# davrempe/humor

Hardware: AMD Instinct MI355X
Metric: fitting closure evaluations/s (stage-3 objective fwd+bwd), batch=32 seq=60 per GPU (higher is better)
Workload: dtype f32

## Files before the change

### humor_amd/csrc/rollout.hip

```cpp
#include <string.h>

#include <algorithm>
#include <list>
#include <unordered_map>
#include <vector>

#include "rollout_persist.h"
#include "rot_math.h"

namespace ha {

constexpr int D_IN = 339, D_STATE = 348, ZD = 48, NJT = 22, NBODY = 21;
template <int ROTW>
struct RawLayout {
  static constexpr int ROOT = 6, RVEL = 6 + ROTW, BODY = 9 + ROTW, JNT = 9 + 22 * ROTW, JVEL = JNT + 66, CONT = JVEL + 66, D = CONT + 9;
};
static_assert(RawLayout<3>::D == 216 && RawLayout<6>::D == 282 && RawLayout<9>::D == 348, "decoder output widths of the three representations");
constexpr int D_INP = 340;
constexpr int SLICE = 64;
constexpr int MAXL = 8;

typedef float f32x16 __attribute__((ext_vector_type(16)));
typedef float vf4 __attribute__((ext_vector_type(4)));

__device__ __forceinline__ size_t qoff(int c) { return (size_t)(c >> 2) * 128 + (c & 3); }

int g_layer_finish = 1;
int g_gemm_rm = 0;
int g_gemm_ks = 2;
int g_rollout_groups = 0;
int g_rollout_persist = 1;
int g_rollout_persist_bwd = 1;
int g_rollout_pipe = 1;
int g_rollout_pipe_bwd = 1;
int g_rollout_persist_inject = 0;

enum class Path : int { chain = 0, one_launch = 1, one_launch_lean = 2 };

struct CallPlan {
  Path path = Path::chain;
  bool piped = false;
  int ngroups = 1, rows_per_group = 0;
  size_t group_floats = 0;
  const float* g_z_add = nullptr;
};

struct PackedLayer {
  int Cin = 0, skip = 0, Nout = 0;
  int nslices_f = 0, main_slices = 0, ntiles_f = 0, Nout_pad = 0;
  int nslices_b = 0, ntiles_b = 0, Nin_pad = 0;
  int group = 0;
  float* Wf = nullptr;
  float* Wb = nullptr;
  float* bias = nullptr;
  float* gamma = nullptr;
  float* beta = nullptr;
};

}

struct ha_humor_net {
  int device = 0;
  int n_dec = 0, n_pri = 0;
  int rotw = 3;
  bool delta = true;
  ha::PackedLayer dec[ha::MAXL], pri[ha::MAXL];
  ha::PersistNet* persist = nullptr;
  struct StashRec { ha::CallPlan plan; int B, S, knobs; std::list<const void*>::iterator age; };
  static constexpr size_t MAX_STASH_RECS = 65536;
  mutable std::unordered_map<const void*, StashRec> stash_recs;
  mutable std::list<const void*> stash_age;
};

namespace ha {

struct LayerTask {
  const float* Wp; const float* bias;
  int ntiles, nslices, main_slices, Nout, Nout_pad;
  const float* src; int nsplit_src; int Csrc;
  const float* skip; int skip_dim;
  int mode;
  const float* gamma; const float* beta; int group; float inv_group;
// ... 253 lines not shown
    v[0] = a0.x; v[1] = a0.y; v[2] = a0.z; v[3] = a0.w; v[4] = a1.x; v[5] = a1.y; v[6] = a1.z; v[7] = a1.w;
  };
  float x[8], da[8];
  if (T.mode == 1) load8(T.src, T.nsplit_src, T.Csrc, x);
  else { load8(T.src, T.nsplit_src, T.Csrc, da); load8(T.hsrc, T.nsplit_h, T.Ch, x); }
  const float gam[8] = {g0.x, g0.y, g0.z, g0.w, g1.x, g1.y, g1.z, g1.w};
  const float bet[8] = {e0.x, e0.y, e0.z, e0.w, e1.x, e1.y, e1.z, e1.w};
  const int per = T.group == SLICE ? 8 : 4, o0 = T.group == SLICE ? 0 : (oct & 4);
  const float inv_n = 1.0f / (float)T.group;
  auto row_sum = [&](int pass, float v) {
    s_red[pass][row][oct] = v;
    __syncthreads();
    float t = 0.f;
    for (int k = 0; k < per; ++k) t += s_red[pass][row][o0 + k];
    return t;
  };
  float p1 = 0.f;
#pragma unroll
  for (int i = 0; i < 8; ++i) p1 += x[i];
  const float mu = row_sum(0, p1) * inv_n;
  float p2 = 0.f;
#pragma unroll
  for (int i = 0; i < 8; ++i) { const float d = x[i] - mu; p2 = fmaf(d, d, p2); }
  const float rstd = rsqrtf(row_sum(1, p2) * inv_n + 1e-5f);
  float out[8];
  if (T.mode == 1) {
#pragma unroll
    for (int i = 0; i < 8; ++i) out[i] = fmaxf((x[i] - mu) * rstd * gam[i] + bet[i], 0.f);
  } else {
    float xh[8], dxh[8], m1 = 0.f, m2 = 0.f;
#pragma unroll
    for (int i = 0; i < 8; ++i) {
      xh[i] = (x[i] - mu) * rstd;
      const float y = xh[i] * gam[i] + bet[i];
      dxh[i] = (y > 0.f ? da[i] : 0.f) * gam[i];
      m1 += dxh[i];
      m2 = fmaf(dxh[i], xh[i], m2);
    }
    m1 = row_sum(2, m1) * inv_n;
    m2 = row_sum(3, m2) * inv_n;
#pragma unroll
    for (int i = 0; i < 8; ++i) out[i] = rstd * (dxh[i] - m1 - xh[i] * m2);
  }
  float* d = F.dst[ti] + (size_t)rt * (T.main_slices * SLICE) * 32 + (size_t)(c0 >> 2) * 128 + (size_t)row * 4;
  *reinterpret_cast<vf4*>(d) = vf4{out[0], out[1], out[2], out[3]};
  *reinterpret_cast<vf4*>(d + 128) = vf4{out[4], out[5], out[6], out[7]};
}


struct GemmTask {
  const float* Wp; const float* bias;
  int ntiles, nslices, Nout;
  const float* src; int Csrc;
  int nrt;
  int epi;
  float slope;
  const float* gamma; const float* beta; int group;
  const float* hsrc; int Ch;
  float* dst_h; float* dst_a; int Cdst;
  int nrg, nwork, per_xcd;
};

constexpr int GEMM_LDS_WAVE = 2 * 8 * 132;

template <int RM, int KS = 1, int TN = 2>
__global__ __launch_bounds__(256) void prior_gemm_kernel(GemmTask T) {
  static_assert(KS == 1 || RM == 1, "the K split is built for one row tile per wave");
  static_assert((KS == 1 || KS == 2 || KS == 4) && (TN == 1 || TN == 2), "prior_gemm_kernel: unsupported shape");
  extern __shared__ __attribute__((aligned(16))) float smem[];
  const int wave = threadIdx.x >> 6, lane = threadIdx.x & 63;
  const int w = (int)(blockIdx.x & 7) * T.per_xcd + (int)(blockIdx.x >> 3);
  if ((int)(blockIdx.x >> 3) >= T.per_xcd || w >= T.nwork) return;
  const int cb = w / T.nrg, rg = w % T.nrg;
  const int kpart = KS == 1 ? 0 : wave % KS;
  const int ct0 = KS == 1 ? (cb * 4 + wave) * TN : (cb * (4 / KS) + wave / KS) * TN;
  const bool tile_ok = ct0 < T.ntiles;
  if (KS == 1 && !tile_ok) return;
  const int ct1 = TN == 2 && ct0 + 1 < T.ntiles ? ct0 + 1 : ct0;
  int rt[RM];
#pragma unroll
  for (int m = 0; m < RM; ++m) rt[m] = rg * RM + m < T.nrt ? rg * RM + m : T.nrt - 1;

  f32x16 acc[RM][TN];
#pragma unroll
  for (int m = 0; m < RM; ++m)
#pragma unroll
    for (int c = 0; c < TN; ++c)
#pragma unroll
      for (int i = 0; i < 16; ++i) acc[m][c][i] = 0.f;

  const float* wp0 = T.Wp + (size_t)ct0 * T.nslices * 2048 + lane * 4;
  const float* wp1 = T.Wp + (size_t)ct1 * T.nslices * 2048 + lane * 4;
  auto load_b = [&](int slice, float (&b0)[32], float (&b1)[32]) {
#pragma unroll
    for (int j = 0; j < 8; ++j) {
      const vf4 u = *reinterpret_cast<const vf4*>(wp0 + (size_t)slice * 2048 + j * 256);
      b0[4 * j] = u.x; b0[4 * j + 1] = u.y; b0[4 * j + 2] = u.z; b0[4 * j + 3] = u.w;
      if (TN == 2) {
        const vf4 v = *reinterpret_cast<const vf4*>(wp1 + (size_t)slice * 2048 + j * 256);
        b1[4 * j] = v.x; b1[4 * j + 1] = v.y; b1[4 * j + 2] = v.z; b1[4 * j + 3] = v.w;
      }
    }
  };
  auto load_a = [&](int slice, float (&a)[RM][32]) {
#pragma unroll
    for (int m = 0; m < RM; ++m)
      load_frag<1>(T.src + (size_t)rt[m] * T.Csrc * 32 + (size_t)(slice * 16 + 8 * (lane >> 5)) * 128 + (size_t)(lane & 31) * 4, 0, 8, a[m]);
  };
  auto mma = [&](const float (&a)[RM][32], const float (&b0)[32], const float (&b1)[32]) {
#pragma unroll
    for (int kp = 0; kp < 32; ++kp)
#pragma unroll
      for (int m = 0; m < RM; ++m) {
        acc[m][0] = __builtin_amdgcn_mfma_f32_32x32x2f32(a[m][kp], b0[kp], acc[m][0], 0, 0, 0);
        if (TN == 2) acc[m][TN - 1] = __builtin_amdgcn_mfma_f32_32x32x2f32(a[m][kp], b1[kp], acc[m][TN - 1], 0, 0, 0);
      }
  };
  const int nfull_all = T.Csrc / SLICE < T.nslices ? T.Csrc / SLICE : T.nslices;
  const int per_part = (nfull_all + KS - 1) / KS;
  const int sbeg = KS == 1 ? 0 : (kpart * per_part < nfull_all ? kpart * per_part : nfull_all);
  const int nfull = KS == 1 ? nfull_all : ((sbeg + per_part) < nfull_all ? (sbeg + per_part) : nfull_all);
  if (nfull > sbeg && (KS == 1 || tile_ok)) {
    float aA[RM][32], bA0[32], bA1[32], aB[RM][32], bB0[32], bB1[32];
    load_b(sbeg, bA0, bA1);
    load_a(sbeg, aA);
    for (int slice = sbeg; slice < nfull; slice += 2) {
      const int s1 = slice + 1 < nfull ? slice + 1 : slice;
      load_b(s1, bB0, bB1);
      load_a(s1, aB);
      HA_SCHED_FENCE();
      mma(aA, bA0, bA1);
      HA_SCHED_FENCE();
      if (slice + 1 < nfull) {
        const int s2 = slice + 2 < nfull ? slice + 2 : slice + 1;
        load_b(s2, bA0, bA1);
        load_a(s2, aA);
        HA_SCHED_FENCE();
        mma(aB, bB0, bB1);
        HA_SCHED_FENCE();
      }
    }
  }
  if (nfull_all < T.nslices && kpart == KS - 1 && (KS == 1 || tile_ok)) {
    float a[RM][32], b0[32], b1[32];
    load_b(nfull_all, b0, b1);
#pragma unroll
    for (int m = 0; m < RM; ++m) load_frag_n<true>(T.src, 1, 0, T.Csrc, rt[m], nfull_all * SLICE, lane, a[m]);
    mma(a, b0, b1);
  }

  float* sl = smem + wave * GEMM_LDS_WAVE;
  const int row = lane & 31, hh = lane >> 5;
  const int ct = hh ? ct0 + 1 : ct0;
  const bool ct_ok = hh < TN && ct < T.ntiles;
  const int hs = hh < TN ? hh : 0;
  float gam[32], bet[32];
  if ((T.epi == 1 || T.epi == 3) && ct_ok) {
#pragma unroll
    for (int j = 0; j < 8; ++j) {
      const vf4 g4 = *reinterpret_cast<const vf4*>(T.gamma + ct * 32 + 4 * j);
      const vf4 b4 = *reinterpret_cast<const vf4*>(T.beta + ct * 32 + 4 * j);
      gam[4 * j] = g4.x; gam[4 * j + 1] = g4.y; gam[4 * j + 2] = g4.z; gam[4 * j + 3] = g4.w;
      bet[4 * j] = b4.x; bet[4 * j + 1] = b4.y; bet[4 * j + 2] = b4.z; bet[4 * j + 3] = b4.w;
    }
  } else {
#pragma unroll
    for (int k = 0; k < 32; ++k) { gam[k] = 1.f; bet[k] = 0.f; }
  }
#pragma unroll
  for (int m = 0; m < RM; ++m) {
#pragma unroll
    for (int c = 0; c < TN; ++c)
#pragma unroll
      for (int i = 0; i < 16; ++i) {
        const int r = (i & 3) + 8 * (i >> 2) + 4 * hh, col = lane & 31;
        sl[(c * 8 + (col >> 2)) * 132 + r * 4 + (col & 3)] = acc[m][c][i];
      }
    if (KS == 1) {
      __builtin_amdgcn_fence(__ATOMIC_RELEASE, "wavefront");
      __builtin_amdgcn_wave_barrier();
      __builtin_amdgcn_fence(__ATOMIC_ACQUIRE, "wavefront");
    } else {
      __syncthreads();
      if (kpart != 0) return;
    }
    float v[32];
#pragma unroll
    for (int j = 0; j < 8; ++j) {
      vf4 q = *reinterpret_cast<const vf4*>(sl + (hs * 8 + j) * 132 + row * 4);
      if (KS > 1) {
#pragma unroll
        for (int pk = 1; pk < KS; ++pk) q += *reinterpret_cast<const vf4*>(sl + pk * GEMM_LDS_WAVE + (hs * 8 + j) * 132 + row * 4);
      }
      v[4 * j] = q.x; v[4 * j + 1] = q.y; v[4 * j + 2] = q.z; v[4 * j + 3] = q.w;
    }
    if (KS == 1) {
      __builtin_amdgcn_fence(__ATOMIC_RELEASE, "wavefront");
      __builtin_amdgcn_wave_barrier();
      __builtin_amdgcn_fence(__ATOMIC_ACQUIRE, "wavefront");
    }
    const bool live = ct_ok && rg * RM + m < T.nrt;
    if (T.bias && ct_ok) {
#pragma unroll
      for (int j = 0; j < 8; ++j) {
        const vf4 b4 = *reinterpret_cast<const vf4*>(T.bias + ct * 32 + 4 * j);
        v[4 * j] += b4.x; v[4 * j + 1] += b4.y; v[4 * j + 2] += b4.z; v[4 * j + 3] += b4.w;
      }
    }
    const size_t o = (size_t)rt[m] * T.Cdst * 32 + (size_t)(ct * 8) * 128 + (size_t)row * 4;
    auto store32 = [&](float* base, const float (&x)[32]) {
#pragma unroll
      for (int j = 0; j < 8; ++j) *reinterpret_cast<vf4*>(base + o + (size_t)j * 128) = vf4{x[4 * j], x[4 * j + 1], x[4 * j + 2], x[4 * j + 3]};
    };
    if (T.epi <= 1 && live) store32(T.dst_h, v);
    if (T.epi == 4) {
#pragma unroll
      for (int k = 0; k < 32; ++k) v[k] = v[k] > 0.f ? v[k] : v[k] * T.slope;
      if (live) store32(T.dst_a, v);
    } else if (T.epi == 5) {
      const float* hp = T.hsrc + (size_t)rt[m] * T.Ch * 32 + (size_t)((ct_ok ? ct : ct0) * 8) * 128 + (size_t)row * 4;
#pragma unroll
      for (int j = 0; j < 8; ++j) {
        const vf4 q = *reinterpret_cast<const vf4*>(hp + (size_t)j * 128);
        v[4 * j] *= q.x > 0.f ? 1.f : T.slope; v[4 * j + 1] *= q.y > 0.f ? 1.f : T.slope;
        v[4 * j + 2] *= q.z > 0.f ? 1.f : T.slope; v[4 * j + 3] *= q.w > 0.f ? 1.f : T.slope;
      }
      if (live) store32(T.dst_a, v);
    } else if (T.epi == 1) {
      const float inv_n = 1.0f / (float)T.group;
      if (T.group == SLICE) gn_apply<1>(1, gam, bet, inv_n, v, v);
      else gn_apply<2>(1, gam, bet, inv_n, v, v);
      if (live) store32(T.dst_a, v);
    } else if (T.epi == 3) {
      float h[32];
      const float* hp = T.hsrc + (size_t)rt[m] * T.Ch * 32 + (size_t)((ct_ok ? ct : ct0) * 8) * 128 + (size_t)row * 4;
#pragma unroll
      for (int j = 0; j < 8; ++j) {
        const vf4 q = *reinterpret_cast<const vf4*>(hp + (size_t)j * 128);
        h[4 * j] = q.x; h[4 * j + 1] = q.y; h[4 * j + 2] = q.z; h[4 * j + 3] = q.w;
      }
      const float inv_n = 1.0f / (float)T.group;
      if (T.group == SLICE) gn_apply<1>(3, gam, bet, inv_n, h, v);
      else gn_apply<2>(3, gam, bet, inv_n, h, v);
      if (live) store32(T.dst_a, v);
    }
  }
}

struct GlueParams {
  int B, S, t, RT;
  const float* xT;
  float* xT_next;
  const float* dec_out; int dec_nsplit; int dec_pad;
  const float* pri_out; int pri_nsplit; int pri_pad;
  const float* Gs;
  float* Gs_next;
  const float* t2j;
  float* world;
  float* prior_mu; float* prior_var;
  const float* g_world;
  const float* g_prior_mu; const float* g_prior_var;
  float* g_dec_out;
  float* g_pri_out;
  const float* gx_dir_in;
  float* gx_dir_out;
  const float* gxp_pri; int gxp_pri_nsplit; int gxp_pri_pad;
  const float* gxp_dec; int gxp_dec_nsplit; int gxp_dec_pad;
  float* carry;
  const float* dz_src[MAXL]; int dz_nsplit[MAXL]; int dz_pad[MAXL]; int dz_off[MAXL]; int dz_n;
  float* g_z;
  float* g_past0;
};

__device__ __forceinline__ float tsum(const float* base, int nsplit, int RT, int C, int rt, int c, int row) {
  return base ? slab_sum(base, nsplit, RT, C, rt, c, row) : 0.f;
}

struct PredState {
  float pj[3], jv[3];
  float dB[9], Bin[9], pB[9];
  float ptrans[3], ptvel[3], prvel[3], dR[9], Rin[9], pR[9];
  float raw_aa_b[9], raw_aa_r[9];
};

template <int ROTW>
__device__ __forceinline__ void delta_rot(const float* raw, float R[9]) {
  if constexpr (ROTW == 3) rodrigues(raw, R);
  else if constexpr (ROTW == 6) rot6d_to_rotmat(raw, R);
  else rot9d_to_rotmat(raw, R);
}
template <int ROTW>
__device__ __forceinline__ void delta_rot_bwd(const float* raw, const float gR[9], float* graw) {
  if constexpr (ROTW == 3) rodrigues_bwd(raw, gR, graw);
  else if constexpr (ROTW == 6) rot6d_to_rotmat_bwd(raw, gR, graw);
  else rot9d_to_rotmat_bwd(raw, gR, graw);
}
// ... 884 lines not shown
      F.t[k] = T;
      F.dst[k] = stash + L.fin[i];
      F.nblk[k] = LL.RT * T.main_slices;
      fb += F.nblk[k];
      T.src = F.dst[k]; T.nsplit_src = 1; T.Csrc = T.main_slices * SLICE; T.mode = 0;
      T.hsrc = nullptr; T.nsplit_h = 0;
    }
    if (fb) {
      HA_LAUNCH(gn_finish_kernel, dim3(fb), dim3(256), 4 * 32 * 8 * sizeof(float), st, F);
      HA_LAUNCH_CHECK();
    }
  }
  LayerTask& T0 = LL.t[0];
  const dim3 grid(T0.ntiles, T0.nsplit_dst, LL.RT);
  T0.nblocks *= LL.RT;
  const bool lean = L.finish && T0.mode == 0 && T0.nsplit_src <= 1;
  if (lean) HA_LAUNCH((mlp_layer_kernel<4, true>), grid, dim3(256), 4 * 1024 * sizeof(float), st, LL);
  else HA_LAUNCH((mlp_layer_kernel<4, false>), grid, dim3(256), 4 * 1024 * sizeof(float), st, LL);
  HA_LAUNCH_CHECK();
  return HA_OK;
}


struct GemmPlan { int rm, tn, ks, ncb; };

static GemmPlan plan_prior_gemm(int ntiles, int nslices, int nrt, int epi, int rm_knob, int ks_knob) {
  GemmPlan P;
  P.ncb = ceil_div(ntiles, 8);
  P.rm = rm_knob == 1 || rm_knob == 2 ? rm_knob : ((nrt / 2) * P.ncb >= 2 * 256 ? 2 : 1);
  P.tn = 2;
  P.ks = 1;
  const bool split_on = ks_knob == 2 || ks_knob == 3;
  if (!split_on || P.rm == 2) return P;
  const bool force = ks_knob == 3;
  if (!force && P.ncb * nrt * 4 > 512) return P;
  const bool gn = epi == 1 || epi == 3;
  constexpr int SIMDS = 1024;
  int best = ceil_div(ceil_div(ntiles, 2) * nrt, SIMDS) * nslices * 2;
  if (force) best = nslices * 2;
  for (int tn = 2; tn >= (gn ? 2 : 1); --tn)
    for (int ks = 1; ks <= 4; ks *= 2) {
      if (ks > 1 && nslices < 2 * ks) continue;
      const int waves = ceil_div(ntiles, tn) * nrt * ks;
      if (!force && waves > 2 * SIMDS) continue;
      const int chain = ceil_div(nslices, ks) * tn;
      const int cost = force ? chain : ceil_div(waves, SIMDS) * chain;
      if (cost < best || (force && cost == best && ks > P.ks)) { best = cost; P.tn = tn; P.ks = ks; P.ncb = ceil_div(ntiles, tn * 4 / ks); }
    }
  return P;
}

static int launch_prior_gemm(GemmTask& T, hipStream_t st) {
  HA_REQUIRE((T.epi != 1 && T.epi != 3) || (T.ntiles % 2 == 0 && (T.group == 32 || T.group == 64)), "prior GEMM: GroupNorm epilogue needs whole 64-column pairs");
  const GemmPlan P = plan_prior_gemm(T.ntiles, T.nslices, T.nrt, T.epi, g_gemm_rm, g_gemm_ks);
  T.nrg = ceil_div(T.nrt, P.rm);
  T.nwork = P.ncb * T.nrg;
  T.per_xcd = ceil_div(T.nwork, 8);
  const dim3 grid(T.per_xcd * 8), block(256);
  const size_t lds = 4 * GEMM_LDS_WAVE * sizeof(float);
  const int shape = P.rm * 100 + P.ks * 10 + P.tn;
  switch (shape) {
    case 212: HA_LAUNCH(prior_gemm_kernel<2>, grid, block, lds, st, T); break;
    case 112: HA_LAUNCH(prior_gemm_kernel<1>, grid, block, lds, st, T); break;
    case 122: HA_LAUNCH((prior_gemm_kernel<1, 2>), grid, block, lds, st, T); break;
    case 142: HA_LAUNCH((prior_gemm_kernel<1, 4>), grid, block, lds, st, T); break;
    case 111: HA_LAUNCH((prior_gemm_kernel<1, 1, 1>), grid, block, lds, st, T); break;
    case 121: HA_LAUNCH((prior_gemm_kernel<1, 2, 1>), grid, block, lds, st, T); break;
    case 141: HA_LAUNCH((prior_gemm_kernel<1, 4, 1>), grid, block, lds, st, T); break;
    default: HA_REQUIRE(false, "prior GEMM: no kernel for RM %d KS %d TN %d", P.rm, P.ks, P.tn);
  }
  HA_LAUNCH_CHECK();
  return HA_OK;
}

static int prior_forward_batched(const ha_humor_net* net, const StashLayout& L, float* stash, int S, hipStream_t st) {
  const int np = net->n_pri;
  for (int l = 0; l < np; ++l) {
    const PackedLayer& P = net->pri[l];
    GemmTask T;
    memset(&T, 0, sizeof(T));
    T.Wp = P.Wf; T.bias = P.bias;
    T.ntiles = P.ntiles_f; T.nslices = P.nslices_f; T.Nout = P.Nout;
    T.src = l == 0 ? stash + L.xT : stash + L.pri_act[(l - 1) & 1];
    T.Csrc = l == 0 ? D_INP : net->pri[l - 1].Nout_pad;
    T.nrt = S * L.RT;
    T.dst_h = stash + L.pri_h[l]; T.Cdst = P.Nout_pad;
    if (l + 1 < np) {
      const PackedLayer& N = net->pri[l + 1];
      T.epi = 1; T.gamma = N.gamma; T.beta = N.beta; T.group = N.group;
      T.dst_a = stash + L.pri_act[l & 1];
    }
    int rc = launch_prior_gemm(T, st);
    if (rc != HA_OK) return rc;
  }
  return HA_OK;
}

static int prior_backward_batched(const ha_humor_net* net, const StashLayout& L, float* stash, int S, hipStream_t st) {
  const int np = net->n_pri;
  for (int l = np - 1; l >= 0; --l) {
    const PackedLayer& P = net->pri[l];
    GemmTask T;
    memset(&T, 0, sizeof(T));
    T.Wp = P.Wb; T.bias = nullptr;
    T.ntiles = P.ntiles_b; T.nslices = P.nslices_b; T.Nout = P.Cin + P.skip;
    T.src = l == np - 1 ? stash + L.g_pri_out : stash + L.pri_act[(l + 1) & 1];
    T.Csrc = P.Nout_pad;
    T.nrt = S * L.RT;
    T.Cdst = P.Nin_pad;
    if (l > 0) {
      T.epi = 3; T.gamma = P.gamma; T.beta = P.beta; T.group = P.group;
      T.hsrc = stash + L.pri_h[l - 1]; T.Ch = net->pri[l - 1].Nout_pad;
      T.dst_a = stash + L.pri_act[l & 1];
    } else {
      T.epi = 0; T.dst_h = stash + L.gx_pri;
    }
    int rc = launch_prior_gemm(T, st);
    if (rc != HA_OK) return rc;
  }
  return HA_OK;
}

constexpr int MAX_GROUPS = 8;

static void group_plan(int B, bool piped, int& ngroups, int& rows_per_group) {
  if (piped) {
    rows_per_group = 256;
    ngroups = ceil_div(B, 256);
    return;
  }
  const int RT = ceil_div(B, 32);
  int n = g_rollout_groups > 0 ? g_rollout_groups : (RT == 2 ? 2 : 1);
  if (n > MAX_GROUPS) n = MAX_GROUPS;
  if (n > RT) n = RT;
  rows_per_group = ceil_div(RT, n) * 32;
  ngroups = ceil_div(B, rows_per_group);
}

static int layout_knobs() { return (g_layer_finish & 3) | ((g_rollout_pipe & 1) << 2) | ((g_rollout_groups & 0xff) << 3); }

static size_t group_stash_floats(const ha_humor_net* net, int rows, int S, bool may_one_launch) {
  StashLayout L;
  make_layout(net, rows, S, Path::chain, L);
// ... 155 lines not shown
  g.B = B; g.S = S; g.t = t; g.RT = RT;
  g.xT = xT;
  g.xT_next = xT + (size_t)RT * D_INP * 32;
  g.dec_out = sp + L.off_dec[nd - 1]; g.dec_nsplit = L.nsf_dec[nd - 1]; g.dec_pad = net->dec[nd - 1].Nout_pad;
  g.Gs = sp + L.off_G;
  g.Gs_next = sp + L.per_step + L.off_G;
  g.t2j = stash + L.t2j;
  g.world = world;
  launch_glue_fwd(net->rotw, net->delta, RT * 32, st, g);
  HA_LAUNCH_CHECK();
  return HA_OK;
}

static int rollout_forward_impl(const ha_humor_net* net, const CallPlan& plan, const StashLayout& L, int B, int S, const float* past_in0,
                                const float* z_seq, float* world, float* prior_mu, float* prior_var, float* stash, hipStream_t st, int phase, int t) {
  const int RT = L.RT, rows = RT * 32;
  auto step_ptr = [&](int t) { return stash + L.steps + (size_t)t * L.per_step; };
  auto x_ptr = [&](int t) { return stash + L.xT + (size_t)t * RT * D_INP * 32; };

  if (L.single) {
    if (phase == PH_BEGIN) {
      PersistFwd f;
      f.B = B; f.S = S;
      f.past_in0 = past_in0; f.z_seq = z_seq; f.world = world;
      f.xT = stash + L.xT; f.steps = stash + L.steps; f.per_step = L.per_step; f.off_G = L.off_G;
      for (int l = 0; l < 4; ++l) f.off_dec[l] = L.off_dec[l];
      for (int l = 0; l < 3; ++l) { f.off_gn[l] = L.off_gn[l]; f.off_ht[l] = L.off_ht[l]; }
      f.off_gl = L.off_gl;
      for (int l = 0; l < 4; ++l) f.dec_pad[l] = net->dec[l].Nout_pad;
      f.hidden_slabs = plan.path != Path::one_launch_lean;
      f.t2j = stash + L.t2j;
      f.ws = stash + L.persist_ws;
      return persist_forward(net->persist, f, ((g_rollout_persist >> 1) & 1) | (g_rollout_persist_inject ? 2 : 0), st);
    }
    if (phase == PH_STEP) return HA_OK;
  }
  if (phase == PH_BEGIN) {
    HA_LAUNCH(transpose_in_kernel, dim3(256), dim3(256), 0, st, z_seq, stash + L.zT, B, S, ZD, ZD, RT);
    HA_LAUNCH_CHECK();
    HA_LAUNCH(transpose_in_kernel, dim3(64), dim3(256), 0, st, past_in0, x_ptr(0), B, 1, D_IN, D_INP, RT);
    HA_LAUNCH_CHECK();
    HA_LAUNCH(init_state_kernel, dim3(ceil_div(rows, 64)), dim3(64), 0, st, past_in0, step_ptr(0) + L.off_G, stash + L.t2j, B, rows);
    HA_LAUNCH_CHECK();
    return HA_OK;
  }

  const int np = net->n_pri;
  if (phase == PH_STEP) {
    GlueParams g;
    memset(&g, 0, sizeof(g));
    return chain_decoder_step(net, L, B, S, t, stash, world, L.hsum, g, st);
  }
  if (prior_mu) {
    int rc = prior_forward_batched(net, L, stash, S, st);
    if (rc != HA_OK) return rc;
    PriorIOParams q;
    memset(&q, 0, sizeof(q));
    q.B = B; q.S = S; q.RT = RT;
    q.pri_pad = net->pri[np - 1].Nout_pad;
    q.pri_out0 = stash + L.pri_h[np - 1]; q.step_stride = (size_t)RT * q.pri_pad * 32; q.pri_nsplit = 1;
    q.prior_mu = prior_mu; q.prior_var = prior_var;
    HA_LAUNCH(prior_io_kernel, dim3(rows, S), dim3(64), 0, st, q);
    HA_LAUNCH_CHECK();
  }
  return HA_OK;
}

extern "C" int ha_humor_rollout_sample(const ha_humor_net* net, int B, int S, const float* past_in0, const float* eps_seq,
                                       float* world, float* prior_mu, float* prior_var, float* z_out, float* stash, void* stream) {
  HA_REQUIRE(net && past_in0 && world && prior_mu && prior_var && z_out && stash, "ha_humor_rollout_sample: null argument");
  HA_REQUIRE(B >= 1 && S >= 1, "ha_humor_rollout_sample: B and S must be >= 1");
  DeviceGuard guard(net->device);
  hipStream_t st = (hipStream_t)stream;
  StashLayout L;
  make_layout(net, B, S, Path::chain, L);
  const int RT = L.RT, rows = RT * 32;
  float* x0 = stash + L.xT;
  HA_LAUNCH(transpose_in_kernel, dim3(64), dim3(256), 0, st, past_in0, x0, B, 1, D_IN, D_INP, RT);
  HA_LAUNCH_CHECK();
  HA_LAUNCH(init_state_kernel, dim3(ceil_div(rows, 64)), dim3(64), 0, st, past_in0, stash + L.steps + L.off_G, stash + L.t2j, B, rows);
  HA_LAUNCH_CHECK();
  const int np = net->n_pri;
  for (int t = 0; t < S; ++t) {
    for (int l = 0; l < np; ++l) {
      LayerLaunch LL;
      memset(&LL, 0, sizeof(LL));
      LL.RT = RT;
      const float* src = l == 0 ? x0 + (size_t)t * RT * D_INP * 32 : stash + L.smp_pri[l - 1];
      fwd_task(LL.t[LL.ntasks++], net->pri[l], src, l == 0 ? 1 : L.nsf_pri[l - 1], nullptr, stash + L.smp_pri[l], L.nsf_pri[l]);
      int rc = launch_layers(LL, L, stash, st);
      if (rc != HA_OK) return rc;
    }
    SampleParams sp_;
    memset(&sp_, 0, sizeof(sp_));
    sp_.B = B; sp_.S = S; sp_.t = t; sp_.RT = RT;
    sp_.pri_out = stash + L.smp_pri[np - 1]; sp_.pri_nsplit = L.nsf_pri[np - 1]; sp_.pri_pad = net->pri[np - 1].Nout_pad;
    sp_.eps = eps_seq; sp_.zT_t = stash + L.zT + (size_t)t * RT * ZD * 32; sp_.z_out = z_out;
    HA_LAUNCH(sample_z_kernel, dim3(rows), dim3(64), 0, st, sp_);
    HA_LAUNCH_CHECK();
    GlueParams g;
    memset(&g, 0, sizeof(g));
    g.pri_out = sp_.pri_out; g.pri_nsplit = sp_.pri_nsplit; g.pri_pad = sp_.pri_pad;
    g.prior_mu = prior_mu; g.prior_var = prior_var;
    int rc = chain_decoder_step(net, L, B, S, t, stash, world, false, g, st);
    if (rc != HA_OK) return rc;
  }
  return HA_OK;
}
// ... 387 lines not shown
  HA_REQUIRE(desc->skip_dim == 0, "ha_mlp_create: skip connections are only supported by the roll-out network");
  HA_REQUIRE(desc->n_linear >= 1 && desc->n_linear <= MAXL, "ha_mlp_create: n_linear=%d out of range", desc->n_linear);
  HA_REQUIRE(act != HA_MLP_LEAKY_RELU || slope > 0.f, "ha_mlp_create: the LeakyReLU slope must be > 0 (the adjoint reads the sign from the activation)");
  DeviceGuard guard(device);
  HA_REQUIRE(guard.ok, "ha_mlp_create: cannot select device %d", device);
  ha_mlp* m = new ha_mlp();
  m->device = device; m->n = desc->n_linear; m->act = act; m->slope = slope;
  m->in_dim = desc->in_dim; m->out_dim = desc->out_dims[desc->n_linear - 1];
  m->in_pad = ceil_div(desc->in_dim, 4) * 4;
  int rc = HA_OK;
  if (act == HA_MLP_GN_RELU) rc = pack_mlp(m->L, desc, "ha_mlp_create");
  else {
    int cin = desc->in_dim;
    for (int i = 0; i < desc->n_linear && rc == HA_OK; ++i) {
      if (!(desc->w[i] && desc->b[i])) { ha::set_error("ha_mlp_create: layer %d weights missing", i); rc = HA_ERR_INVALID_ARG; break; }
      rc = pack_layer(m->L[i], desc->w[i], desc->b[i], nullptr, nullptr, cin, 0, desc->out_dims[i], false);
      cin = desc->out_dims[i];
    }
  }
  if (rc != HA_OK) { ha_mlp_destroy(m); return rc; }
  for (int i = 0; i < m->n; ++i) {
    if (m->L[i].Nout_pad > m->wmax) m->wmax = m->L[i].Nout_pad;
    if (m->L[i].Nin_pad > m->wmax) m->wmax = m->L[i].Nin_pad;
  }
  *out = m;
  return HA_OK;
}

extern "C" int ha_mlp_destroy(ha_mlp* m) {
  if (!m) return HA_OK;
  DeviceGuard guard(m->device);
  for (int i = 0; i < MAXL; ++i) {
    PackedLayer& P = m->L[i];
    float* ptrs[5] = {P.Wf, P.Wb, P.bias, P.gamma, P.beta};
    for (float* p : ptrs)
      if (p) (void)hipFree(p);
  }
  delete m;
  return HA_OK;
}

extern "C" int ha_mlp_workspace(const ha_mlp* m, int N, int64_t* ws_floats) {
  HA_REQUIRE(m && ws_floats && N >= 1, "ha_mlp_workspace: bad argument");
  *ws_floats = (int64_t)mlp_layout(m, N).total;
  return HA_OK;
}

extern "C" int ha_mlp_forward(const ha_mlp* m, int N, const float* x, int tail, float* y, float* ws, void* stream) {
  HA_REQUIRE(m && x && y && ws && N >= 1, "ha_mlp_forward: bad argument");
  HA_REQUIRE(tail == HA_MLP_TAIL_NONE || (tail == HA_MLP_TAIL_ROT6D_AA && m->out_dim % 6 == 0), "ha_mlp_forward: tail %d needs an output width that is a multiple of 6", tail);
  DeviceGuard guard(m->device);
  hipStream_t st = (hipStream_t)stream;
  const MlpLayout W = mlp_layout(m, N);
  HA_LAUNCH(transpose_in_kernel, dim3(ceil_div((int)((size_t)W.nrt * m->in_pad * 32), 256)), dim3(256), 0, st, x, ws + W.xT, N, 1, m->in_dim,
                     m->in_pad, W.nrt);
  HA_LAUNCH_CHECK();
  for (int l = 0; l < m->n; ++l) {
    const PackedLayer& P = m->L[l];
    const bool last = l + 1 == m->n;
    GemmTask T;
    memset(&T, 0, sizeof(T));
    T.Wp = P.Wf; T.bias = P.bias;
    T.ntiles = P.ntiles_f; T.nslices = P.nslices_f; T.Nout = P.Nout;
    T.nrt = W.nrt; T.Cdst = P.Nout_pad;
    T.Csrc = l == 0 ? m->in_pad : m->L[l - 1].Nout_pad;
    if (m->act == HA_MLP_LEAKY_RELU) {
      T.src = l == 0 ? ws + W.xT : ws + W.keep[l - 1];
      if (last) { T.epi = 0; T.dst_h = ws + W.out; }
      else { T.epi = 4; T.slope = m->slope; T.dst_a = ws + W.keep[l]; }
    } else {
      T.src = l == 0 ? ws + W.xT : ws + W.pp[(l - 1) & 1];
      if (last) { T.epi = 0; T.dst_h = ws + W.out; }
      else {
        const PackedLayer& Nx = m->L[l + 1];
        T.epi = 1; T.gamma = Nx.gamma; T.beta = Nx.beta; T.group = Nx.group;
        T.dst_h = ws + W.keep[l]; T.dst_a = ws + W.pp[l & 1];
      }
    }
    int rc = launch_prior_gemm(T, st);
    if (rc != HA_OK) return rc;
  }
  const int C = m->out_dim, Cpad = m->L[m->n - 1].Nout_pad;
  const size_t items = tail == HA_MLP_TAIL_NONE ? (size_t)N * C : (size_t)N * (C / 6);
  HA_LAUNCH(mlp_out_kernel, dim3((unsigned)ceil_div((int)items, 256)), dim3(256), 0, st, ws + W.out, y, N, C, Cpad, tail);
  HA_LAUNCH_CHECK();
  return HA_OK;
}

extern "C" int ha_mlp_backward(const ha_mlp* m, int N, const float* g_y, int tail, float* ws, float* g_x, void* stream) {
  HA_REQUIRE(m && g_y && g_x && ws && N >= 1, "ha_mlp_backward: bad argument");
  HA_REQUIRE(tail == HA_MLP_TAIL_NONE || (tail == HA_MLP_TAIL_ROT6D_AA && m->out_dim % 6 == 0), "ha_mlp_backward: tail %d needs an output width that is a multiple of 6", tail);
  DeviceGuard guard(m->device);
  hipStream_t st = (hipStream_t)stream;
  const MlpLayout W = mlp_layout(m, N);
  const int C = m->out_dim, Cpad = m->L[m->n - 1].Nout_pad;
  float* g_out = ws + W.pp[(m->n - 1) & 1];
  const size_t items = tail == HA_MLP_TAIL_NONE ? (size_t)W.nrt * 32 * Cpad : (size_t)W.nrt * 32 * ceil_div(Cpad, 6);
  HA_LAUNCH(mlp_gout_kernel, dim3((unsigned)ceil_div((int)items, 256)), dim3(256), 0, st, g_y, ws + W.out, g_out, N, W.nrt, C, Cpad, tail);
  HA_LAUNCH_CHECK();
  for (int l = m->n - 1; l >= 0; --l) {
    const PackedLayer& P = m->L[l];
    GemmTask T;
    memset(&T, 0, sizeof(T));
    T.Wp = P.Wb; T.bias = nullptr;
    T.ntiles = P.ntiles_b; T.nslices = P.nslices_b; T.Nout = P.Cin;
    T.src = ws + W.pp[l & 1]; T.Csrc = P.Nout_pad;
    T.nrt = W.nrt; T.Cdst = P.Nin_pad;
    if (l == 0) { T.epi = 0; T.dst_h = ws + W.gx; }
    else {
      T.hsrc = ws + W.keep[l - 1]; T.Ch = m->L[l - 1].Nout_pad;
      T.dst_a = ws + W.pp[(l - 1) & 1];
      if (m->act == HA_MLP_LEAKY_RELU) { T.epi = 5; T.slope = m->slope; }
      else { T.epi = 3; T.gamma = P.gamma; T.beta = P.beta; T.group = P.group; }
    }
    int rc = launch_prior_gemm(T, st);
    if (rc != HA_OK) return rc;
  }
  HA_LAUNCH(mlp_out_kernel, dim3((unsigned)ceil_div((int)((size_t)N * m->in_dim), 256)), dim3(256), 0, st, ws + W.gx, g_x, N, m->in_dim,
                     m->L[0].Nin_pad, 0);
  HA_LAUNCH_CHECK();
  return HA_OK;
}
```

### humor_amd/csrc/smpl.hip

```cpp
#include <stdarg.h>
#include <string.h>
#include <algorithm>

#include <vector>

#include "smpl_model.h"
#ifndef HA_SIMT_EMU
#include "lane_reduce.h"
#endif

namespace ha {

static thread_local char g_err[512] = "";
void set_error(const char* fmt, ...) {
  va_list ap;
  va_start(ap, fmt);
  vsnprintf(g_err, sizeof(g_err), fmt, ap);
  va_end(ap);
}

}

namespace ha {
int g_skin_variant = -1;
int g_dense_gA_sparse = 2;
int g_dense_bwd_waves = 0;
extern int g_layer_finish, g_gemm_rm, g_rollout_groups, g_gemm_ks, g_rollout_persist, g_rollout_persist_bwd, g_rollout_persist_inject, g_rollout_pipe, g_rollout_pipe_bwd;
extern unsigned g_cu_poison;
}
extern "C" int ha_tune_set(const char* key, int value) {
  HA_REQUIRE(key, "ha_tune_set: null key");
  if (strcmp(key, "skin_variant") == 0) { ha::g_skin_variant = value; return HA_OK; }
  if (strcmp(key, "dense_bwd_waves") == 0) { ha::g_dense_bwd_waves = value; return HA_OK; }
  if (strcmp(key, "dense_gA_sparse") == 0) { ha::g_dense_gA_sparse = value; return HA_OK; }
  if (strcmp(key, "layer_finish") == 0) { ha::g_layer_finish = value; return HA_OK; }
  if (strcmp(key, "gemm_rm") == 0) { ha::g_gemm_rm = value; return HA_OK; }
  if (strcmp(key, "rollout_groups") == 0) { ha::g_rollout_groups = value; return HA_OK; }
  if (strcmp(key, "gemm_ks") == 0) { ha::g_gemm_ks = value; return HA_OK; }
  if (strcmp(key, "rollout_persist") == 0) { ha::g_rollout_persist = value; return HA_OK; }
  if (strcmp(key, "rollout_persist_bwd") == 0) { ha::g_rollout_persist_bwd = value; return HA_OK; }
  if (strcmp(key, "rollout_pipe") == 0) { ha::g_rollout_pipe = value; return HA_OK; }
  if (strcmp(key, "rollout_pipe_bwd") == 0) { ha::g_rollout_pipe_bwd = value; return HA_OK; }
  if (strcmp(key, "rollout_persist_inject") == 0) { ha::g_rollout_persist_inject = value; return HA_OK; }
  if (strcmp(key, "cu_poison") == 0) { ha::g_cu_poison = (unsigned)value; return HA_OK; }
  ha::set_error("ha_tune_set: unknown key '%s'", key);
  return HA_ERR_INVALID_ARG;
}
extern "C" const char* ha_last_error(void) { return ha::g_err; }
extern "C" int ha_abi_version(void) { return 3; }
extern "C" int ha_device_arch(int device, char* buf, int buflen) {
  HA_REQUIRE(buf && buflen > 0, "ha_device_arch: null buffer");
  hipDeviceProp_t prop;
  HA_CHECK_HIP(hipGetDeviceProperties(&prop, device));
  snprintf(buf, buflen, "%s", prop.gcnArchName);
  return HA_OK;
}

namespace ha {

template <typename T>
static int upload(T** dst, const std::vector<T>& src) {
  *dst = nullptr;
  if (src.empty()) return HA_OK;
  HA_CHECK_HIP(hipMalloc((void**)dst, src.size() * sizeof(T)));
  HA_CHECK_HIP(hipMemcpy(*dst, src.data(), src.size() * sizeof(T), hipMemcpyHostToDevice));
  return HA_OK;
}

static void free_set(VertexSet& s) {
  if (s.Pd_v) (void)hipFree(s.Pd_v);
  if (s.Pd_k) (void)hipFree(s.Pd_k);
  if (s.w) (void)hipFree(s.w);
  if (s.idx) (void)hipFree(s.idx);
  if (s.Wc) (void)hipFree(s.Wc);
  if (s.ids) (void)hipFree(s.ids);
  s = VertexSet();
}

static int build_set(ha_smpl_model* m, int slot, const int32_t* ids, int n) {
  VertexSet& s = m->sets[slot];
  free_set(s);
  s.n = n;
  s.nchunks = ceil_div(n, kChunk);
  s.npad = s.nchunks * kChunk;
  const int K = m->Kfull, V = m->V, nnz = m->nnz;
  std::vector<float> pd((size_t)s.nchunks * K * 3 * kChunk, 0.0f);
  const int Kp = ceil_div(K, 128) * 128;
  std::vector<float> pdk((size_t)s.nchunks * 3 * kChunk * Kp, 0.0f);
  std::vector<float> w((size_t)s.nchunks * nnz * kChunk, 0.0f);
  std::vector<int32_t> ix((size_t)s.nchunks * nnz * kChunk, 0);
  std::vector<float> wc((size_t)s.nchunks * kChunk * kMaxJoints, 0.0f);
// ... 1894 lines not shown
```

Before: 625.4.

## Fold layout transposes and output scatter into prior GEMM epilogues

After: 638.2, median of 6. +2.0%, better.

```diff
diff --git a/humor_amd/csrc/rollout.hip b/humor_amd/csrc/rollout.hip
--- a/humor_amd/csrc/rollout.hip
+++ b/humor_amd/csrc/rollout.hip
@@ -1,3 +1,4 @@
+#include <stdint.h>
 #include <string.h>
 
 #include <algorithm>
@@ -22,12 +23,14 @@
 
 typedef float f32x16 __attribute__((ext_vector_type(16)));
 typedef float vf4 __attribute__((ext_vector_type(4)));
+typedef float vf2 __attribute__((ext_vector_type(2)));
 
 __device__ __forceinline__ size_t qoff(int c) { return (size_t)(c >> 2) * 128 + (c & 3); }
 
 int g_layer_finish = 1;
 int g_gemm_rm = 0;
 int g_gemm_ks = 2;
+int g_gemm_fold = 1;
 int g_rollout_groups = 0;
 int g_rollout_persist = 1;
 int g_rollout_persist_bwd = 1;
@@ -387,6 +390,7 @@
   const float* Wp; const float* bias;
   int ntiles, nslices, Nout;
   const float* src; int Csrc;
+  int src_rows;
   int nrt;
   int epi;
   float slope;
@@ -394,6 +398,8 @@
   const float* hsrc; int Ch;
   float* dst_h; float* dst_a; int Cdst;
   int nrg, nwork, per_xcd;
+  float* rm_dst; float* rm_dst2;
+  int rm_RT, rm_S, rm_rows, rm_w, rm_C, rm_split, rm_vec2;
 };
 
 constexpr int GEMM_LDS_WAVE = 2 * 8 * 132;
@@ -416,6 +422,50 @@
 #pragma unroll
   for (int m = 0; m < RM; ++m) rt[m] = rg * RM + m < T.nrt ? rg * RM + m : T.nrt - 1;
 
+  const int row = lane & 31, hh = lane >> 5;
+  const int ct = hh ? ct0 + 1 : ct0;
+  const bool ct_ok = hh < TN && ct < T.ntiles;
+  const int hs = hh < TN ? hh : 0;
+  float gam[32], bet[32], bia[32], hpre[RM][32];
+  auto load_affine = [&]() {
+    if ((T.epi == 1 || T.epi == 3) && ct_ok) {
+#pragma unroll
+      for (int j = 0; j < 8; ++j) {
+        const vf4 g4 = *reinterpret_cast<const vf4*>(T.gamma + ct * 32 + 4 * j);
+        const vf4 b4 = *reinterpret_cast<const vf4*>(T.beta + ct * 32 + 4 * j);
+        gam[4 * j] = g4.x; gam[4 * j + 1] = g4.y; gam[4 * j + 2] = g4.z; gam[4 * j + 3] = g4.w;
+        bet[4 * j] = b4.x; bet[4 * j + 1] = b4.y; bet[4 * j + 2] = b4.z; bet[4 * j + 3] = b4.w;
+      }
+    } else {
+#pragma unroll
+      for (int k = 0; k < 32; ++k) { gam[k] = 1.f; bet[k] = 0.f; }
+    }
+  };
+  auto load_bias = [&]() {
+    if (T.bias && ct_ok) {
+#pragma unroll
+      for (int j = 0; j < 8; ++j) {
+        const vf4 b4 = *reinterpret_cast<const vf4*>(T.bias + ct * 32 + 4 * j);
+        bia[4 * j] = b4.x; bia[4 * j + 1] = b4.y; bia[4 * j + 2] = b4.z; bia[4 * j + 3] = b4.w;
+      }
+    } else {
+#pragma unroll
+      for (int k = 0; k < 32; ++k) bia[k] = 0.f;
+    }
+  };
+  auto load_h = [&](int m) {
+    if (T.epi == 3 || T.epi == 5) {
+      const float* hp = T.hsrc + (size_t)rt[m] * T.Ch * 32 + (size_t)((ct_ok ? ct : (tile_ok ? ct0 : 0)) * 8) * 128 + (size_t)row * 4;
+#pragma unroll
+      for (int j = 0; j < 8; ++j) {
+        const vf4 q = *reinterpret_cast<const vf4*>(hp + (size_t)j * 128);
+        hpre[m][4 * j] = q.x; hpre[m][4 * j + 1] = q.y; hpre[m][4 * j + 2] = q.z; hpre[m][4 * j + 3] = q.w;
+      }
+    } else {
+#pragma unroll
+      for (int k = 0; k < 32; ++k) hpre[m][k] = 0.f;
+    }
+  };
   f32x16 acc[RM][TN];
 #pragma unroll
   for (int m = 0; m < RM; ++m)
@@ -451,7 +501,7 @@
         if (TN == 2) acc[m][TN - 1] = __builtin_amdgcn_mfma_f32_32x32x2f32(a[m][kp], b1[kp], acc[m][TN - 1], 0, 0, 0);
       }
   };
-  const int nfull_all = T.Csrc / SLICE < T.nslices ? T.Csrc / SLICE : T.nslices;
+  const int nfull_all = T.src_rows > 0 ? 0 : (T.Csrc / SLICE < T.nslices ? T.Csrc / SLICE : T.nslices);
   const int per_part = (nfull_all + KS - 1) / KS;
   const int sbeg = KS == 1 ? 0 : (kpart * per_part < nfull_all ? kpart * per_part : nfull_all);
   const int nfull = KS == 1 ? nfull_all : ((sbeg + per_part) < nfull_all ? (sbeg + per_part) : nfull_all);
@@ -479,29 +529,26 @@
   if (nfull_all < T.nslices && kpart == KS - 1 && (KS == 1 || tile_ok)) {
     float a[RM][32], b0[32], b1[32];
     load_b(nfull_all, b0, b1);
-#pragma unroll
-    for (int m = 0; m < RM; ++m) load_frag_n<true>(T.src, 1, 0, T.Csrc, rt[m], nfull_all * SLICE, lane, a[m]);
+    if (T.src_rows > 0) {
+#pragma unroll
+      for (int m = 0; m < RM; ++m) {
+        const int r = rt[m] * 32 + (lane & 31);
+#pragma unroll
+        for (int kp = 0; kp < 32; ++kp) {
+          const int c = 32 * (lane >> 5) + kp;
+          const bool ok = r < T.src_rows && c < T.Csrc;
+          const float x = T.src[ok ? (size_t)r * T.Csrc + c : 0];
+          a[m][kp] = ok ? x : 0.f;
+        }
+      }
+    } else {
+#pragma unroll
+      for (int m = 0; m < RM; ++m) load_frag_n<true>(T.src, 1, 0, T.Csrc, rt[m], nfull_all * SLICE, lane, a[m]);
+    }
     mma(a, b0, b1);
   }
 
   float* sl = smem + wave * GEMM_LDS_WAVE;
-  const int row = lane & 31, hh = lane >> 5;
-  const int ct = hh ? ct0 + 1 : ct0;
-  const bool ct_ok = hh < TN && ct < T.ntiles;
-  const int hs = hh < TN ? hh : 0;
-  float gam[32], bet[32];
-  if ((T.epi == 1 || T.epi == 3) && ct_ok) {
-#pragma unroll
-    for (int j = 0; j < 8; ++j) {
-      const vf4 g4 = *reinterpret_cast<const vf4*>(T.gamma + ct * 32 + 4 * j);
-      const vf4 b4 = *reinterpret_cast<const vf4*>(T.beta + ct * 32 + 4 * j);
-      gam[4 * j] = g4.x; gam[4 * j + 1] = g4.y; gam[4 * j + 2] = g4.z; gam[4 * j + 3] = g4.w;
-      bet[4 * j] = b4.x; bet[4 * j + 1] = b4.y; bet[4 * j + 2] = b4.z; bet[4 * j + 3] = b4.w;
-    }
-  } else {
-#pragma unroll
-    for (int k = 0; k < 32; ++k) { gam[k] = 1.f; bet[k] = 0.f; }
-  }
 #pragma unroll
   for (int m = 0; m < RM; ++m) {
 #pragma unroll
@@ -511,6 +558,13 @@
         const int r = (i & 3) + 8 * (i >> 2) + 4 * hh, col = lane & 31;
         sl[(c * 8 + (col >> 2)) * 132 + r * 4 + (col & 3)] = acc[m][c][i];
       }
+    if (m == 0 && kpart == 0) {
+      load_affine();
+      load_bias();
+#pragma unroll
+      for (int mm = 0; mm < RM; ++mm) load_h(mm);
+      HA_SCHED_FENCE();
+    }
     if (KS == 1) {
       __builtin_amdgcn_fence(__ATOMIC_RELEASE, "wavefront");
       __builtin_amdgcn_wave_barrier();
@@ -537,29 +591,53 @@
     const bool live = ct_ok && rg * RM + m < T.nrt;
     if (T.bias && ct_ok) {
 #pragma unroll
-      for (int j = 0; j < 8; ++j) {
-        const vf4 b4 = *reinterpret_cast<const vf4*>(T.bias + ct * 32 + 4 * j);
-        v[4 * j] += b4.x; v[4 * j + 1] += b4.y; v[4 * j + 2] += b4.z; v[4 * j + 3] += b4.w;
-      }
+      for (int k = 0; k < 32; ++k) v[k] += bia[k];
     }
     const size_t o = (size_t)rt[m] * T.Cdst * 32 + (size_t)(ct * 8) * 128 + (size_t)row * 4;
     auto store32 = [&](float* base, const float (&x)[32]) {
 #pragma unroll
       for (int j = 0; j < 8; ++j) *reinterpret_cast<vf4*>(base + o + (size_t)j * 128) = vf4{x[4 * j], x[4 * j + 1], x[4 * j + 2], x[4 * j + 3]};
     };
-    if (T.epi <= 1 && live) store32(T.dst_h, v);
+    if (T.epi <= 1 && live && T.dst_h) store32(T.dst_h, v);
+    if (T.rm_dst && live) {
+      const int tile = rg * RM + m, t = tile / T.rm_RT, r = (tile - t * T.rm_RT) * 32 + row;
+      if (r < T.rm_rows) {
+        const size_t line = ((size_t)r * T.rm_S + t) * T.rm_w;
+        float* const d0 = T.rm_dst + line;
+        float* const d1 = T.rm_dst2 ? T.rm_dst2 + line - T.rm_split : d0;
+        float x[32];
+        if (T.rm_dst2) {
+#pragma unroll
+          for (int k = 0; k < 32; ++k) {
+            const float e = expf(v[k]), p = v[k] + 0.f;
+            x[k] = ct * 32 + k >= T.rm_split ? e : p;
+          }
+        } else {
+#pragma unroll
+          for (int k = 0; k < 32; ++k) x[k] = v[k];
+        }
+        if (T.rm_vec2) {
+#pragma unroll
+          for (int k = 0; k < 32; k += 2) {
+            const int c = ct * 32 + k;
+            if (c < T.rm_C) *reinterpret_cast<vf2*>((c >= T.rm_split ? d1 : d0) + c) = vf2{x[k], x[k + 1]};
+          }
+        } else {
+#pragma unroll
+          for (int k = 0; k < 32; ++k) {
+            const int c = ct * 32 + k;
+            if (c < T.rm_C) (c >= T.rm_split ? d1 : d0)[c] = x[k];
+          }
+        }
+      }
+    }
     if (T.epi == 4) {
 #pragma unroll
       for (int k = 0; k < 32; ++k) v[k] = v[k] > 0.f ? v[k] : v[k] * T.slope;
       if (live) store32(T.dst_a, v);
     } else if (T.epi == 5) {
-      const float* hp = T.hsrc + (size_t)rt[m] * T.Ch * 32 + (size_t)((ct_ok ? ct : ct0) * 8) * 128 + (size_t)row * 4;
-#pragma unroll
-      for (int j = 0; j < 8; ++j) {
-        const vf4 q = *reinterpret_cast<const vf4*>(hp + (size_t)j * 128);
-        v[4 * j] *= q.x > 0.f ? 1.f : T.slope; v[4 * j + 1] *= q.y > 0.f ? 1.f : T.slope;
-        v[4 * j + 2] *= q.z > 0.f ? 1.f : T.slope; v[4 * j + 3] *= q.w > 0.f ? 1.f : T.slope;
-      }
+#pragma unroll
+      for (int k = 0; k < 32; ++k) v[k] *= hpre[m][k] > 0.f ? 1.f : T.slope;
       if (live) store32(T.dst_a, v);
     } else if (T.epi == 1) {
       const float inv_n = 1.0f / (float)T.group;
@@ -567,16 +645,9 @@
       else gn_apply<2>(1, gam, bet, inv_n, v, v);
       if (live) store32(T.dst_a, v);
     } else if (T.epi == 3) {
-      float h[32];
-      const float* hp = T.hsrc + (size_t)rt[m] * T.Ch * 32 + (size_t)((ct_ok ? ct : ct0) * 8) * 128 + (size_t)row * 4;
-#pragma unroll
-      for (int j = 0; j < 8; ++j) {
-        const vf4 q = *reinterpret_cast<const vf4*>(hp + (size_t)j * 128);
-        h[4 * j] = q.x; h[4 * j + 1] = q.y; h[4 * j + 2] = q.z; h[4 * j + 3] = q.w;
-      }
       const float inv_n = 1.0f / (float)T.group;
-      if (T.group == SLICE) gn_apply<1>(3, gam, bet, inv_n, h, v);
-      else gn_apply<2>(3, gam, bet, inv_n, h, v);
+      if (T.group == SLICE) gn_apply<1>(3, gam, bet, inv_n, hpre[m], v);
+      else gn_apply<2>(3, gam, bet, inv_n, hpre[m], v);
       if (live) store32(T.dst_a, v);
     }
   }
@@ -1567,6 +1638,12 @@
 
 static int launch_prior_gemm(GemmTask& T, hipStream_t st) {
   HA_REQUIRE((T.epi != 1 && T.epi != 3) || (T.ntiles % 2 == 0 && (T.group == 32 || T.group == 64)), "prior GEMM: GroupNorm epilogue needs whole 64-column pairs");
+  HA_REQUIRE(!T.rm_dst || (T.epi == 0 && T.rm_RT >= 1 && T.rm_C <= T.ntiles * 32 && (T.rm_dst2 || T.rm_split >= T.rm_C)), "prior GEMM: bad row-major destination");
+  HA_REQUIRE(T.src_rows == 0 || (T.nslices == 1 && T.Csrc <= SLICE && T.src_rows <= T.nrt * 32), "prior GEMM: a row-major A operand is one K slice");
+  if (T.rm_dst) {
+    auto odd = [](const void* q) { return ((uintptr_t)q & 7) != 0; };
+    T.rm_vec2 = !(((T.rm_w | T.rm_C | T.rm_split) & 1) || odd(T.rm_dst) || (T.rm_dst2 && odd(T.rm_dst2)));
+  }
   const GemmPlan P = plan_prior_gemm(T.ntiles, T.nslices, T.nrt, T.epi, g_gemm_rm, g_gemm_ks);
   T.nrg = ceil_div(T.nrt, P.rm);
   T.nwork = P.ncb * T.nrg;
@@ -1588,7 +1665,8 @@
   return HA_OK;
 }
 
-static int prior_forward_batched(const ha_humor_net* net, const StashLayout& L, float* stash, int S, hipStream_t st) {
+static int prior_forward_batched(const ha_humor_net* net, const StashLayout& L, float* stash, int B, int S, float* prior_mu, float* prior_var,
+                                 hipStream_t st) {
   const int np = net->n_pri;
   for (int l = 0; l < np; ++l) {
     const PackedLayer& P = net->pri[l];
@@ -1604,6 +1682,9 @@
       const PackedLayer& N = net->pri[l + 1];
       T.epi = 1; T.gamma = N.gamma; T.beta = N.beta; T.group = N.group;
       T.dst_a = stash + L.pri_act[l & 1];
+    } else if (prior_mu) {
+      T.rm_dst = prior_mu; T.rm_dst2 = prior_var;
+      T.rm_RT = L.RT; T.rm_S = S; T.rm_rows = B; T.rm_w = ZD; T.rm_split = ZD; T.rm_C = 2 * ZD;
     }
     int rc = launch_prior_gemm(T, st);
     if (rc != HA_OK) return rc;
@@ -1865,8 +1946,10 @@
     return chain_decoder_step(net, L, B, S, t, stash, world, L.hsum, g, st);
   }
   if (prior_mu) {
-    int rc = prior_forward_batched(net, L, stash, S, st);
+    const bool fold = g_gemm_fold != 0 && net->pri[np - 1].Nout == 2 * ZD;
+    int rc = prior_forward_batched(net, L, stash, B, S, fold ? prior_mu : nullptr, fold ? prior_var : nullptr, st);
     if (rc != HA_OK) return rc;
+    if (fold) return HA_OK;
     PriorIOParams q;
     memset(&q, 0, sizeof(q));
     q.B = B; q.S = S; q.RT = RT;
@@ -2360,9 +2443,14 @@
   DeviceGuard guard(m->device);
   hipStream_t st = (hipStream_t)stream;
   const MlpLayout W = mlp_layout(m, N);
-  HA_LAUNCH(transpose_in_kernel, dim3(ceil_div((int)((size_t)W.nrt * m->in_pad * 32), 256)), dim3(256), 0, st, x, ws + W.xT, N, 1, m->in_dim,
-                     m->in_pad, W.nrt);
-  HA_LAUNCH_CHECK();
+  const int C = m->out_dim, Cpad = m->L[m->n - 1].Nout_pad;
+  const bool fold_y = g_gemm_fold != 0 && tail == HA_MLP_TAIL_NONE;
+  const bool fold_x = g_gemm_fold != 0 && m->in_dim <= SLICE;
+  if (!fold_x) {
+    HA_LAUNCH(transpose_in_kernel, dim3(ceil_div((int)((size_t)W.nrt * m->in_pad * 32), 256)), dim3(256), 0, st, x, ws + W.xT, N, 1, m->in_dim,
+                       m->in_pad, W.nrt);
+    HA_LAUNCH_CHECK();
+  }
   for (int l = 0; l < m->n; ++l) {
     const PackedLayer& P = m->L[l];
     const bool last = l + 1 == m->n;
@@ -2385,10 +2473,15 @@
         T.dst_h = ws + W.keep[l]; T.dst_a = ws + W.pp[l & 1];
       }
     }
+    if (l == 0 && fold_x) { T.src = x; T.Csrc = m->in_dim; T.src_rows = N; }
+    if (last && fold_y) {
+      T.dst_h = nullptr;
+      T.rm_dst = y; T.rm_RT = W.nrt; T.rm_S = 1; T.rm_rows = N; T.rm_w = T.rm_C = T.rm_split = C;
+    }
     int rc = launch_prior_gemm(T, st);
     if (rc != HA_OK) return rc;
   }
-  const int C = m->out_dim, Cpad = m->L[m->n - 1].Nout_pad;
+  if (fold_y) return HA_OK;
   const size_t items = tail == HA_MLP_TAIL_NONE ? (size_t)N * C : (size_t)N * (C / 6);
   HA_LAUNCH(mlp_out_kernel, dim3((unsigned)ceil_div((int)items, 256)), dim3(256), 0, st, ws + W.out, y, N, C, Cpad, tail);
   HA_LAUNCH_CHECK();
@@ -2414,8 +2507,11 @@
     T.ntiles = P.ntiles_b; T.nslices = P.nslices_b; T.Nout = P.Cin;
     T.src = ws + W.pp[l & 1]; T.Csrc = P.Nout_pad;
     T.nrt = W.nrt; T.Cdst = P.Nin_pad;
-    if (l == 0) { T.epi = 0; T.dst_h = ws + W.gx; }
-    else {
+    if (l == 0) {
+      T.epi = 0;
+      if (g_gemm_fold != 0) { T.rm_dst = g_x; T.rm_RT = W.nrt; T.rm_S = 1; T.rm_rows = N; T.rm_w = T.rm_C = T.rm_split = m->in_dim; }
+      else T.dst_h = ws + W.gx;
+    } else {
       T.hsrc = ws + W.keep[l - 1]; T.Ch = m->L[l - 1].Nout_pad;
       T.dst_a = ws + W.pp[(l - 1) & 1];
       if (m->act == HA_MLP_LEAKY_RELU) { T.epi = 5; T.slope = m->slope; }
@@ -2424,6 +2520,7 @@
     int rc = launch_prior_gemm(T, st);
     if (rc != HA_OK) return rc;
   }
+  if (g_gemm_fold != 0) return HA_OK;
   HA_LAUNCH(mlp_out_kernel, dim3((unsigned)ceil_div((int)((size_t)N * m->in_dim), 256)), dim3(256), 0, st, ws + W.gx, g_x, N, m->in_dim,
                      m->L[0].Nin_pad, 0);
   HA_LAUNCH_CHECK();
diff --git a/humor_amd/csrc/smpl.hip b/humor_amd/csrc/smpl.hip
--- a/humor_amd/csrc/smpl.hip
+++ b/humor_amd/csrc/smpl.hip
@@ -25,7 +25,7 @@
 int g_skin_variant = -1;
 int g_dense_gA_sparse = 2;
 int g_dense_bwd_waves = 0;
-extern int g_layer_finish, g_gemm_rm, g_rollout_groups, g_gemm_ks, g_rollout_persist, g_rollout_persist_bwd, g_rollout_persist_inject, g_rollout_pipe, g_rollout_pipe_bwd;
+extern int g_layer_finish, g_gemm_rm, g_rollout_groups, g_gemm_ks, g_gemm_fold, g_rollout_persist, g_rollout_persist_bwd, g_rollout_persist_inject, g_rollout_pipe, g_rollout_pipe_bwd;
 extern unsigned g_cu_poison;
 }
 extern "C" int ha_tune_set(const char* key, int value) {
@@ -37,6 +37,7 @@
   if (strcmp(key, "gemm_rm") == 0) { ha::g_gemm_rm = value; return HA_OK; }
   if (strcmp(key, "rollout_groups") == 0) { ha::g_rollout_groups = value; return HA_OK; }
   if (strcmp(key, "gemm_ks") == 0) { ha::g_gemm_ks = value; return HA_OK; }
+  if (strcmp(key, "gemm_fold") == 0) { ha::g_gemm_fold = value; return HA_OK; }
   if (strcmp(key, "rollout_persist") == 0) { ha::g_rollout_persist = value; return HA_OK; }
   if (strcmp(key, "rollout_persist_bwd") == 0) { ha::g_rollout_persist_bwd = value; return HA_OK; }
   if (strcmp(key, "rollout_pipe") == 0) { ha::g_rollout_pipe = value; return HA_OK; }
```
